# skmhrk1209/VSRD

Measured on AMD Instinct MI355X. Metric: rendered rays/sec (fwd+bwd) per GPU, KITTI-360 376×1408, 16 instances, higher is better.
Workload: dtype f32

## Files before the change

vsrd_amd/csrc/api.hip:

```cpp
#include <cstdio>
#include <cstdlib>
#include "../../include/vsrd_hip.h"
#include "aux_kernels.h"
#include "quad_step.h"
#include "matching.h"
#include "ray_sampling.h"
#include "projection.h"
#include "frame_step.h"
#include "hypernetwork.h"
#include "frame_ingest.h"
#include "frame_labels.h"
#include "frame_group_labels.h"
#include "frame_masks.h"
#include "frame_metrics.h"
#include "frame_log.h"
#include "patch_correlation.h"
#include "launch.h"

namespace {

using namespace vsrd;

constexpr int kMaxBlocks = 16384;

// ... 783 lines not shown
    const bool split = !r.rows && !(config->flags & VSRD_FLAG_STEP_WAVE_PER_RAY) && !wants_samples(config) && (rounds == 2 || rounds == 4) &&
                       (force_split || config->num_rays <= switches().split_max_rays) &&
                       static_cast<size_t>(split_lds_floats(S, N)) * sizeof(float) <= kLdsLimit / 2;
    if (split) {
        const int blocks = config->num_rays < kSplitBlocks ? config->num_rays : kSplitBlocks;
        const int num_waves = blocks * kPairWaves;
        if (static_cast<size_t>(num_waves) * (row + 1) * sizeof(float) > workspace_bytes) return VSRD_E_WORKSPACE;
        if (frames.count > 1 && static_cast<long long>(workspace_bytes) > frames.stride) return VSRD_E_INVALID_ARGUMENT;
        const size_t lds_bytes = static_cast<size_t>(split_lds_floats(S, N)) * sizeof(float);
        const FieldArgs f = field_args(field);
        RenderArgs c = render_args(config);
        c.sh.inv_t = f.inv_t;
        float* partials = static_cast<float*>(workspace);
        float* loss_partials = partials + static_cast<size_t>(num_waves) * row;
        int32_t status = VSRD_OK;
        for_rounds<2, 4>(rounds, [&](auto k) {
            for_bool(frames.count > 1 || header, [&](auto batch) {
                constexpr auto kernel = render_silhouette_split_kernel<decltype(k)::value, decltype(batch)::value>;
                if ((status = opt_in_lds(kernel, lds_bytes)) != VSRD_OK) return;
                hipLaunchKernelGGL(kernel, dim3(blocks, frames.count), dim3(kPairWaves * kWave), lds_bytes, s, f, field->instances, c, origins, directions, u_coarse,
                                   u_fine, targets, instance_weights, loss_scale, labels, partials, loss_partials, header);
            });
        });
        if (status != VSRD_OK) return status;
        if (launch_status() != VSRD_OK) return VSRD_E_LAUNCH;
        hipLaunchKernelGGL(reduce_partials_kernel, dim3(row + 1, frames.count), dim3(256), 0, s, partials, num_waves, row, grad_instances, nullptr, loss_partials, 1, loss,
                           frames.stride, header);
        return launch_status();
    }
    if (frames.count > 1 || header) return VSRD_E_UNSUPPORTED;
    Geometry g;
    if (!plan(r.rows ? static_cast<int>(r.num_groups) : config->num_rays, r.rows ? r.lds_floats : static_cast<size_t>(wave_lds_floats(S, N)) + N + row, &g))
        return VSRD_E_UNSUPPORTED;
#ifdef VSRD_INSTANCE_LDS
    if (r.quad && r.full) g.lds_bytes += static_cast<size_t>(N) * kInstanceStride * sizeof(float);
#endif
    if (!cap_to_workspace(vsrd_workspace_bytes(N, 0), row + 1, r.flag_bytes, &g)) return VSRD_E_WORKSPACE;
    const FieldArgs f = field_args(field);
    RenderArgs c = render_args(config);
    c.sh.inv_t = f.inv_t;
    const int num_waves = g.blocks * (g.threads / kWave);
    float* partials = static_cast<float*>(workspace);
    float* loss_partials = partials + static_cast<size_t>(num_waves) * row;
    unsigned char* redo_flags = reinterpret_cast<unsigned char*>(loss_partials + num_waves);
    int32_t status = VSRD_OK;
    bool known = true;
    if (r.rows) {
        auto launch = [&](auto hot, auto rest) {
            if ((status = opt_in_lds(hot, g.lds_bytes)) != VSRD_OK || (status = opt_in_lds(rest, g.lds_bytes)) != VSRD_OK) return;
            if (hipMemsetAsync(redo_flags, 0, 16, s) != hipSuccess) { status = VSRD_E_LAUNCH; return; }
            launch_hot_then_rest(hot, rest, g, s, f, field->instances, c, origins, directions, u_coarse, u_fine, targets, instance_weights, loss_scale, labels, partials,
                                 loss_partials, redo_flags);
        };
        if (r.quad && r.full) launch(render_silhouette_quad_kernel<4, true, true>, render_silhouette_quad_kernel<4, false, false>);
        else if (r.full) launch(render_silhouette_pair_kernel<4, true, true>, render_silhouette_pair_kernel<4, false, false>);
        else if (r.quad) known = for_rounds<1, 2, 4>(r.rounds, [&](auto k) {
            launch(render_silhouette_quad_kernel<decltype(k)::value, true, false>, render_silhouette_quad_kernel<decltype(k)::value, false, false>); });
        else known = for_rounds<2, 4>(r.rounds, [&](auto k) {
            launch(render_silhouette_pair_kernel<decltype(k)::value, true, false>, render_silhouette_pair_kernel<decltype(k)::value, false, false>); });
    } else {
        known = for_rounds<1, 2, 4>(rounds, [&](auto k) {
            constexpr auto kernel = render_silhouette_kernel<decltype(k)::value>;
            if ((status = opt_in_lds(kernel, g.lds_bytes)) != VSRD_OK) return;
            hipLaunchKernelGGL(kernel, dim3(g.blocks), dim3(g.threads), g.lds_bytes, s, f, field->instances, c, origins, directions, u_coarse, u_fine, targets,
                               instance_weights, loss_scale, labels, partials, loss_partials);
        });
    }
    if (!known) return VSRD_E_UNSUPPORTED;
    if (status != VSRD_OK) return status;
    if (launch_status() != VSRD_OK) return VSRD_E_LAUNCH;
    hipLaunchKernelGGL(reduce_partials_kernel, dim3(row + 1), dim3(256), 0, s, partials, num_waves, row, grad_instances, nullptr, loss_partials, 1, loss);
    return launch_status();
}

static int32_t residual_step_single_kernel(const vsrd_field* field, const vsrd_render_config* config,
                                  const float* origins, const float* directions, const float* u_coarse, const float* u_fine,
                                  const float* targets, const float* instance_weights, float loss_scale, float eikonal_ratio,
                                  void* workspace, size_t workspace_bytes,
                                  float* losses, float* grad_instances, float* grad_mlp_weights, float* labels, void* stream) {
    if (!valid_field(field) || !valid_config(config, true) || !workspace || !losses || !grad_instances || !grad_mlp_weights) return VSRD_E_INVALID_ARGUMENT;
    if (field->mlp_weights == nullptr) return VSRD_E_INVALID_ARGUMENT;
    const int N = field->num_instances;
    if (workspace_bytes < vsrd_workspace_bytes(N, 1)) return VSRD_E_WORKSPACE;
    const hipStream_t s = static_cast<hipStream_t>(stream);
    const int row = N * kGradStride, mlp_row = N * kMlpWeights;
    if (config->num_rays == 0) {
        if (hipMemsetAsync(losses, 0, 2 * sizeof(float), s) != hipSuccess) return VSRD_E_LAUNCH;
        if (hipMemsetAsync(grad_mlp_weights, 0, mlp_row * sizeof(float), s) != hipSuccess) return VSRD_E_LAUNCH;
        return hipMemsetAsync(grad_instances, 0, row * sizeof(float), s) == hipSuccess ? VSRD_OK : VSRD_E_LAUNCH;
    }
    if (!origins || !directions || !targets) return VSRD_E_INVALID_ARGUMENT;
    const int S = config->num_samples;
    const int num_points = 2 * S - 1;
    const int rounds = rounds_for(num_points);
    Geometry g;
    if (!plan(config->num_rays, static_cast<size_t>(residual_step_lds_floats(S, N)), &g)) return VSRD_E_UNSUPPORTED;
    if (g.threads > kResidualWaves * kWave) return VSRD_E_UNSUPPORTED;
    if (g.blocks > kMaxBlocksResidual) g.blocks = kMaxBlocksResidual;
    const FieldArgs f = field_args(field);
    RenderArgs c = render_args(config);
    c.sh.inv_t = f.inv_t;
    const int num_waves = g.blocks * (g.threads / kWave);
    const OneKernelWorkspace w = one_kernel_workspace(workspace, N, true);
    float* loss_partials = w.partials + static_cast<size_t>(num_waves) * row;
    const float eikonal_norm = 1.0f / (static_cast<float>(config->num_rays) * static_cast<float>(num_points));
    const float eikonal_scale = eikonal_ratio * eikonal_norm;
    int32_t status = VSRD_OK;
    const bool known = for_rounds<1, 2, 4>(rounds, [&](auto k) {
// ... 674 lines not shown
```

vsrd_amd/csrc/quad_step.h:

```cpp
#pragma once
#include "render_kernels.h"

namespace vsrd {

constexpr int kQuadRays = 4;
constexpr int kRowLanes = 16;
constexpr int kQuadMaxInstances = 16;
constexpr int kQuadMaxSamples = 64;
constexpr int kPairMaxInstances = 64;
constexpr int kPairMaxSamples = 128;

constexpr int kDppRowShl1 = 0x101, kDppRowShl2 = 0x102, kDppRowShl4 = 0x104, kDppRowShl8 = 0x108;

__device__ __forceinline__ float max_xor16(float v) {
    float a = v, b = v;
    asm volatile("s_nop 1\n\tv_permlane16_swap_b32 %0, %1" : "+v"(a), "+v"(b));
    return fmaxf(a, b);
}
__device__ __forceinline__ float lane_gather(float v, int byte_address) {
    return __builtin_bit_cast(float, __builtin_amdgcn_ds_bpermute(byte_address, __builtin_bit_cast(int, v)));
}

struct RowLanes {
    int lane, row, col;
// ... 169 lines not shown
        }
    }
    if (u_fine == nullptr) {
        const float inv_total = fast_rcp(running + extra_spacing);
#pragma unroll
        for (int k = 0; k < kRoundsS; ++k) {
            const int idx = k * kL + rl.col;
            if (idx < S) {
                const float sorted_u = fminf(spacing[k] * inv_total, 0.99999994f);
                usorted[idx] = sorted_u;
                if (u_fine_out != nullptr && write) u_fine_out[urow + idx] = sorted_u;
            }
        }
    }
    wave_lds_sync();
    if (u_fine != nullptr && !sorted_input) {
#pragma unroll
        for (int k = 0; k < kRoundsS; ++k) {
            if (k * kL >= S) continue;
            const int idx = k * kL + rl.col;
            const bool valid = idx < S;
            const float v = uraw[valid ? idx : 0];
            int rank = 0;
            for (int j = 0; j < S; ++j) {
                const float o = uraw[j];
                rank += ((o < v) || (o == v && j < idx)) ? 1 : 0;
            }
            if (valid) usorted[rank] = v;
        }
        wave_lds_sync();
    }
}

template <bool kStrict>
__device__ __forceinline__ int count_below_64(const float* a, int n, float v) {
    int pos = 0;
#pragma unroll
    for (int stride = 32; stride >= 1; stride >>= 1) {
        const float probe = a[min(pos + stride - 1, n - 1)];
        pos += (kStrict ? (probe < v) : (probe <= v)) ? stride : 0;
    }
    const float probe = a[min(pos, n - 1)];
    pos += (kStrict ? (probe < v) : (probe <= v)) ? 1 : 0;
    return min(pos, n);
}

template <int kL, bool kStrict>
__device__ __forceinline__ int seg_count_below(const float* a, int n, float v) {
    if (kL == kRowLanes) return count_below_64<kStrict>(a, n, v);
    return count_below<kStrict>(a, n, v, search_iterations(n));
}

template <int kL, int kRoundsS>
__device__ __forceinline__ void quad_importance_merge(float* rowbase, int S, const float (&w)[kRoundsS], const RowLanes& rl) {
    float* coarse = rowbase;
    float* fine = rowbase + S;
    float* merged = rowbase + quad_merged_offset(S, kL);
    float* cdf = merged + S;
    float total = 0.0f;
#pragma unroll
    for (int k = 0; k < kRoundsS; ++k) total += seg_sum<kL>(fabsf(w[k]));
    const float denom = fmaxf(total, 1.0e-12f);
    float running = 0.0f;
#pragma unroll
    for (int k = 0; k < kRoundsS; ++k) {
        if (k * kL >= S - 1) continue;
        const int idx = k * kL + rl.col;
        const float inclusive = seg_inclusive_sum<kL>(w[k] / denom) + running;
        if (idx < S - 1) cdf[idx + 1] = inclusive;
        running = lane_gather(inclusive, rl.last);
    }
    if (rl.col == 0) cdf[0] = 0.0f;
    wave_lds_sync();
    float fine_max = -3.0e38f;
#pragma unroll
    for (int k = 0; k < kRoundsS; ++k) {
        if (k * kL >= S) continue;
        const int j = k * kL + rl.col;
        const bool valid = j < S;
        const float u = fine[valid ? j : (S - 1)];
        int upper = seg_count_below<kL, true>(cdf, S, u);
        upper = min(max(upper, 1), S - 1);
        const float c_lo = cdf[upper - 1], c_hi = cdf[upper];
        const float b_lo = coarse[upper - 1], b_hi = coarse[upper];
        const float t = (u - c_lo) / (c_hi - c_lo + 1.0e-6f);
        float sample = torch_lerp(b_lo, b_hi, t);
        const float scan = seg_inclusive_max<kL>(valid ? sample : -3.0e38f);
        sample = fmaxf(scan, fine_max);
        fine_max = fmaxf(fine_max, lane_gather(scan, rl.last));
        wave_lds_sync();
        if (valid) fine[j] = sample;
    }
    wave_lds_sync();
#pragma unroll
    for (int k = 0; k < kRoundsS; ++k) {
        if (k * kL >= S) continue;
        const int j = k * kL + rl.col;
        const bool valid = j < S;
        const int jj = valid ? j : (S - 1);
        const float a = coarse[jj], b = fine[jj];
        const int rank_a = jj + seg_count_below<kL, true>(fine, S, a);
        const int rank_b = jj + seg_count_below<kL, false>(coarse, S, b);
        if (valid) { merged[rank_a] = a; merged[rank_b] = b; }
    }
    wave_lds_sync();
}

struct RowRay { Ray ray; float reach; };
__device__ __forceinline__ RowRay load_row_ray(const float* rp) {
    const float4 a = *reinterpret_cast<const float4*>(rp), b = *reinterpret_cast<const float4*>(rp + 4);
    RowRay r;
    r.ray.ox = a.x; r.ray.oy = a.y; r.ray.oz = a.z; r.ray.rx = a.w; r.ray.ry = b.x; r.ray.rz = b.y; r.reach = b.z;
    return r;
}
__device__ __forceinline__ RayCull row_cull(const float* coef, const RowRay& r) {
    RayCull rc;
    rc.coef = coef;
    rc.c2 = r.ray.rx * r.ray.rx + r.ray.ry * r.ray.ry + r.ray.rz * r.ray.rz;
    rc.rnorm = fast_sqrt(rc.c2);
    rc.reach = r.reach;
    return rc;
}
__device__ __forceinline__ void reload_fence() { asm volatile("" ::: "memory"); }

template <int kL>
__device__ __forceinline__ void quad_ray_setup(const float* __restrict__ instances, int N, int padded, const Ray& r, float* coef, float* rayp, const RowLanes& rl) {
    float amax = 0.0f;
    for (int i = rl.col; i < padded; i += kL) {
        const bool real = i < N;
        const float* p = instances + (real ? i : 0) * kInstanceStride;
        const float ex = r.ox - p[0], ey = r.oy - p[1], ez = r.oz - p[2];
        const float a = ex * ex + ey * ey + ez * ez;
        coef[kCullCoefs * i + 0] = real ? a : 3.0e38f;
        coef[kCullCoefs * i + 1] = real ? 2.0f * (ex * r.rx + ey * r.ry + ez * r.rz) : 0.0f;
        coef[kCullCoefs * i + 2] = real ? fast_sqrt(p[12] * p[12] + p[13] * p[13] + p[14] * p[14]) * (1.0f / (1.0f - kCullSlack)) : 0.0f;
        coef[kCullCoefs * i + 3] = 0.0f;
        amax = fmaxf(amax, real ? a : 0.0f);
    }
    const float reach = fast_sqrt(fmaxf(seg_max<kL>(amax), r.ox * r.ox + r.oy * r.oy + r.oz * r.oz));
    if (rl.col == 0) {
        *reinterpret_cast<float4*>(rayp) = make_float4(r.ox, r.oy, r.oz, r.rx);
        *reinterpret_cast<float4*>(rayp + 4) = make_float4(r.ry, r.rz, reach, 0.0f);
    }
    wave_lds_sync();
}

// ... 286 lines not shown
#endif
            int slot = 0;
            for (unsigned long long todo = st.near[q]; todo != 0ull; todo &= todo - 1ull, ++slot) {
                const int i = __builtin_ctzll(todo);
                if (!((lam_any >> i) & 1ull)) continue;
                acc += coef_own[kCullCoefs * i + 3] * quad_cached_term<(kL > kRowLanes), false, kYaw>(instances, i, slot, cbuf, rl.lane, p.x, p.y, p.z, st.m[q], sh.inv_t);
            }
        } else {
            for (unsigned long long todo = st.near[q] & lam_any; todo != 0ull; todo &= todo - 1ull) {
                const int i = __builtin_ctzll(todo);
                const Instance in = load_instance_block(instances, i);
                acc += coef_own[kCullCoefs * i + 3] * fast_exp(-(box_value<kYaw>(in, p.x, p.y, p.z).d - st.m[q]) * sh.inv_t);
            }
        }
        const float lam_z = p.valid ? acc * st.inv_z[q] : 0.0f;
        UnionValue v;
        v.u = st.m[q] + st.s[q]; v.gx = st.ax[q]; v.gy = st.ay[q]; v.gz = st.az[q];
        const Opacity op = opacity_of(v, rr.ray, p.delta, sh);
        const float alpha = p.valid ? op.alpha : 0.0f;
        const float t = trans_mid[q * kL + rl.col];
        trans_mid[q * kL + rl.col] = p.mid;
        const float wgt = t * alpha;
        const float contrib = lam_z * wgt;
        const float suffix_inclusive = seg_suffix_sum<kL>(contrib, rl);
        const float Q = suffix_inclusive - contrib + suffix_carry;
        suffix_carry += lane_gather(suffix_inclusive, rl.first);
        const float alpha_bar = lam_z * t - Q * fast_rcp(1.0f - alpha);
        const float x_bar = (p.valid && op.xx > 0.0f) ? alpha_bar : 0.0f;
        const float inv_pe = fast_rcp(op.phi_p + sh.eps);
        const float phi_p_bar = x_bar * (op.phi_n + sh.eps) * inv_pe * inv_pe;
        const float phi_n_bar = -x_bar * inv_pe;
        const float sp_bar = phi_p_bar * op.phi_p * (1.0f - op.phi_p) * sh.inv_std;
        const float sn_bar = phi_n_bar * op.phi_n * (1.0f - op.phi_n) * sh.inv_std;
        const float u_bar = sp_bar + sn_bar;
        const float cprime_bar = (sn_bar - sp_bar) * p.delta / 2.0f;
        const float slope = (1.0f - sh.ratio) * ((0.5f - 0.5f * op.cosine > 0.0f) ? 0.5f : 0.0f) + sh.ratio * ((-op.cosine > 0.0f) ? 1.0f : 0.0f);
        const float cos_bar = cprime_bar * slope;
        const float nbx = cos_bar * rr.ray.rx, nby = cos_bar * rr.ray.ry, nbz = cos_bar * rr.ray.rz;
        const float n_dot = op.nx * nbx + op.ny * nby + op.nz * nbz;
        const float gbx = (nbx - op.nx * n_dot) * op.inv_gn, gby = (nby - op.ny * n_dot) * op.inv_gn, gbz = (nbz - op.nz * n_dot) * op.inv_gn;
        const float B = cos_bar * st.c[q];
        const float A = gbx * st.ax[q] + gby * st.ay[q] + gbz * st.az[q];
        st.ax[q] = gbx; st.ay[q] = gby; st.az[q] = gbz;
        st.s[q] = 1.0f + st.s[q] * sh.inv_t;
        c2buf[q * kL + rl.col + 1] = sh.inv_t * (A + wgt * lam_z);
        cbuf[(2 * q) * kWave + rl.lane] = u_bar + sh.inv_t * B;
        cbuf[(2 * q + 1) * kWave + rl.lane] = sh.inv_t * wgt;
        const bool any = (u_bar != 0.0f) || (gbx != 0.0f) || (gby != 0.0f) || (gbz != 0.0f) || (wgt != 0.0f);
        flow |= (__ballot(any) != 0ull) ? (1u << q) : 0u;
    }
    return flow;
}

template <int kL, int kRounds, bool kYaw>
__device__ __forceinline__ void quad_phase_b(const QuadAdjoint<kRounds>& st, const float* __restrict__ instances, const Shading& sh, const float* rayp,
                                             unsigned flow, const float* coef_own, const float* cbuf, const float* mids, const float* c2buf, float (&G)[kL == kRowLanes ? 4 : 16], const RowLanes& rl) {
    const float inv_t = sh.inv_t;
    const Ray ray = load_row_ray(rayp).ray;
    unsigned long long todo = 0ull;
#pragma unroll
    for (int q = 0; q < kRounds; ++q) todo |= ((flow >> q) & 1u) ? st.near[q] : 0ull;
    for (; todo != 0ull; todo &= todo - 1ull) {
        const int i = __builtin_ctzll(todo);
        const Instance in = load_instance_block(instances, i);
        const float lam_i = coef_own[kCullCoefs * i + 3];
        float at0 = 0, at1 = 0, at2 = 0, ad0 = 0, ad1 = 0, ad2 = 0;
        float r00 = 0, r01 = 0, r02 = 0, r10 = 0, r11 = 0, r12 = 0, r20 = 0, r21 = 0, r22 = 0;
#pragma unroll
        for (int q = 0; q < kRounds; ++q) {
            if (!(((st.near[q] >> i) & 1ull) && ((flow >> q) & 1u))) continue;
            const float mid = mids[q * kL + rl.col];
            const float c1 = cbuf[(2 * q) * kWave + rl.lane], c3 = cbuf[(2 * q + 1) * kWave + rl.lane], c2 = c2buf[q * kL + rl.col + 1];
#ifndef VSRD_BOUND_FREE_SELECTORS
            const BoxEval e = eval_box<kYaw>(in, ray.ox + ray.rx * mid, ray.oy + ray.ry * mid, ray.oz + ray.rz * mid);
#else
            BoxEval e = box_value<kYaw>(in, ray.ox + ray.rx * mid, ray.oy + ray.ry * mid, ray.oz + ray.rz * mid);
            e.hx = fmaxf(e.qx, 0.0f) * e.inv; e.hy = fmaxf(e.qy, 0.0f) * e.inv; e.hz = fmaxf(e.qz, 0.0f) * e.inv;
            e.glx = __builtin_copysignf(e.hx, e.px); e.gly = __builtin_copysignf(e.hy, e.py); e.glz = __builtin_copysignf(e.hz, e.pz);
#endif
            const float ds = e.d - st.m[q];
            const float w = fast_exp(-ds * inv_t) * st.inv_z[q];
            const float cc = w * (st.s[q] - ds * inv_t);
            const float gx_ = st.ax[q], gy_ = st.ay[q], gz_ = st.az[q];
            const float rgx = kYaw ? fmaf(in.r20, gz_, in.r00 * gx_) : fmaf(in.r20, gz_, fmaf(in.r10, gy_, in.r00 * gx_));
            const float rgy = kYaw ? gy_ : fmaf(in.r21, gz_, fmaf(in.r11, gy_, in.r01 * gx_));
            const float rgz = kYaw ? fmaf(in.r22, gz_, in.r02 * gx_) : fmaf(in.r22, gz_, fmaf(in.r12, gy_, in.r02 * gx_));
            const float tb = inv_t * (rgx * e.glx + rgy * e.gly + rgz * e.glz);
            const float d_bar = cc * (c1 - tb) + w * (c2 - tb - c3 * lam_i);
            const float gwbx = cc * gx_, gwby = cc * gy_, gwbz = cc * gz_;
            const float glbx = cc * rgx, glby = cc * rgy, glbz = cc * rgz;
#ifndef VSRD_BOUND_FREE_SELECTORS
            const float sx = sign_of(e.px), sy = sign_of(e.py), sz = sign_of(e.pz);
#else
            const float sx = __builtin_copysignf(1.0f, e.px), sy = __builtin_copysignf(1.0f, e.py), sz = __builtin_copysignf(1.0f, e.pz);
#endif
            const float vx = sx * glbx, vy = sy * glby, vz = sz * glbz;
            const float inv_n = box_inverse_norm(e);
            const float hx = fmaxf(e.qx, 0.0f) * inv_n, hy = fmaxf(e.qy, 0.0f) * inv_n, hz = fmaxf(e.qz, 0.0f) * inv_n;
            const float hv = hx * vx + hy * vy + hz * vz;
#ifndef VSRD_BOUND_FREE_SELECTORS
            const float qbx = d_bar * e.hx + ((e.qx > 0.0f) ? (vx - hx * hv) * inv_n : 0.0f);
            const float qby = d_bar * e.hy + ((e.qy > 0.0f) ? (vy - hy * hv) * inv_n : 0.0f);
            const float qbz = d_bar * e.hz + ((e.qz > 0.0f) ? (vz - hz * hv) * inv_n : 0.0f);
#else
            const float qbx = d_bar * e.hx + (vx - hx * hv) * inv_n;
            const float qby = d_bar * e.hy + (vy - hy * hv) * inv_n;
            const float qbz = d_bar * e.hz + (vz - hz * hv) * inv_n;
#endif
            const float pbx = sx * qbx, pby = sy * qby, pbz = sz * qbz;
            ad0 -= qbx; ad1 -= qby; ad2 -= qbz;
            r00 += e.relx * pbx + gwbx * e.glx; r02 += e.relx * pbz + gwbx * e.glz;
            r20 += e.relz * pbx + gwbz * e.glx; r22 += e.relz * pbz + gwbz * e.glz;
            if (!(kYaw && sh.yaw_gradients)) {
                r01 += e.relx * pby + gwbx * e.gly;
                r10 += e.rely * pbx + gwby * e.glx; r11 += e.rely * pby + gwby * e.gly; r12 += e.rely * pbz + gwby * e.glz;
                r21 += e.relz * pby + gwbz * e.gly;
            }
            if (kYaw) {
                at0 -= in.r00 * pbx + in.r02 * pbz; at1 -= pby; at2 -= in.r20 * pbx + in.r22 * pbz;
            } else {
                at0 -= in.r00 * pbx + in.r01 * pby + in.r02 * pbz;
                at1 -= in.r10 * pbx + in.r11 * pby + in.r12 * pbz;
                at2 -= in.r20 * pbx + in.r21 * pby + in.r22 * pbz;
            }
        }
        const float packed[16] = {at0, at1, at2, r00, r01, r02, r10, r11, r12, r20, r21, r22, ad0, ad1, ad2, 0.0f};
        const float mine = wave_reduce16_scatter(packed, rl.lane);
        const float add = ((rl.lane >> 4) == (i & 3)) ? mine : 0.0f;
        if (kL == kRowLanes) {
#pragma unroll
            for (int s = 0; s < 4; ++s) G[s] += ((i >> 2) == s) ? add : 0.0f;
        } else {
            switch (i >> 2) {
#define VSRD_G_CASE(s) case s: G[s] += add; break;
                VSRD_G_CASE(0) VSRD_G_CASE(1) VSRD_G_CASE(2) VSRD_G_CASE(3) VSRD_G_CASE(4) VSRD_G_CASE(5) VSRD_G_CASE(6) VSRD_G_CASE(7)
                VSRD_G_CASE(8) VSRD_G_CASE(9) VSRD_G_CASE(10) VSRD_G_CASE(11) VSRD_G_CASE(12) VSRD_G_CASE(13) VSRD_G_CASE(14) VSRD_G_CASE(15)
#undef VSRD_G_CASE
                default: break;
            }
        }
    }
}

#ifdef VSRD_PHASE_TIMERS
#define VSRD_QUAD_CLOCK_PARAM , PhaseClock& phase_clock
#define VSRD_QUAD_CLOCK_ARG , phase_clock
#else
#define VSRD_QUAD_CLOCK_PARAM
#define VSRD_QUAD_CLOCK_ARG
#endif

template <int kL, int kRoundsS, bool kYaw, bool kRunning>
__device__ __forceinline__ bool quad_step_body(const float* __restrict__ instances, int N, int NP, const RenderArgs& c, const Shading& sh, int first_ray,
                                               const float* __restrict__ origins, const float* __restrict__ directions,
                                               const float* __restrict__ u_coarse, const float* __restrict__ u_fine, bool sorted_input,
                                               const float* __restrict__ targets, const float* __restrict__ instance_weights, float loss_scale,
                                               float* __restrict__ labels_out, float* stage, float* dcache, float* coefs, float* rays,
                                               float (&G)[kL == kRowLanes ? 4 : 16], float& loss_acc, const RowLanes& rl VSRD_QUAD_CLOCK_PARAM) {
    constexpr int kRounds = 2 * kRoundsS;
    constexpr int kSlots = kL == kRowLanes ? 1 : 2;
    VSRD_PHASE(7);
    const int S = c.num_samples;
    const int num_points = 2 * S - 1;
    const int my_ray = first_ray + rl.row;
    const bool alive = my_ray < c.num_rays;
    const int ray = alive ? my_ray : (c.num_rays - 1);
    const long long src = source_row(c, ray);
    float* rowbase = stage + rl.row * quad_row_floats(S, kL);
    float* coef_own = coefs + rl.row * quad_coef_floats(NP);
    const unsigned long long real = NP > N ? ((1ull << N) - 1ull) : ~0ull;
    {
        const long long origin_row = (c.ray_indices && c.rays_per_origin > 0) ? src / c.rays_per_origin : src;
        const float* o = origins + origin_row * c.origin_stride;
        const float* d = directions + src * 3;
        Ray r;
        r.ox = o[0]; r.oy = o[1]; r.oz = o[2]; r.rx = d[0]; r.ry = d[1]; r.rz = d[2];
        quad_ray_setup<kL>(instances, N, NP, r, coef_own, rays + rl.row * kRowRayFloats, rl);
    }
    quad_stage_samples<kL, kRoundsS>(rowbase, c, S, ray, u_coarse, u_fine, sorted_input, rl, c.out_u_coarse, c.out_u_fine, alive);
    VSRD_PHASE(0);
    float w1[kRoundsS];
    if (!quad_pass_one<kL, kRoundsS, kYaw, kRunning>(instances, NP, sh, rays + rl.row * kRowRayFloats, coef_own, rowbase, S, w1, rl, real)) return false;
    VSRD_PHASE(1);
    if (c.out_coarse_weights != nullptr && alive) {
#pragma unroll
        for (int k = 0; k < kRoundsS; ++k)
            if (k * kL + rl.col < S - 1) c.out_coarse_weights[static_cast<size_t>(my_ray) * (S - 1) + k * kL + rl.col] = w1[k];
    }
    float coarse_total = 0.0f;
#pragma unroll
    for (int k = 0; k < kRoundsS; ++k) coarse_total += seg_sum<kL>(w1[k]);
    const bool live = alive && !((c.flags & 2u) && coarse_total == 0.0f);
    const unsigned long long live_lanes = __ballot(live);
    float label[kSlots];
#pragma unroll
    for (int s = 0; s < kSlots; ++s) label[s] = 0.0f;
    unsigned active = 0u;
    int cached_round = -1;
    QuadAdjoint<kRounds> st;
    const int data_row = live ? rl.row : (live_lanes != 0ull ? (__builtin_ctzll(live_lanes) / kL) : rl.row);
    const float* rayp = rays + data_row * kRowRayFloats;
    const float* merged = stage + data_row * quad_row_floats(S, kL) + quad_merged_offset(S, kL);
    float* trans_mid = rowbase;
    if (live_lanes != 0ull) {
        quad_importance_merge<kL, kRoundsS>(rowbase, S, w1, rl);
        if (c.out_distances != nullptr && live) {
            float* dst = c.out_distances + static_cast<size_t>(my_ray) * (2 * S);
            const float* own = rowbase + quad_merged_offset(S, kL);
            for (int idx = rl.col; idx < 2 * S; idx += kL) dst[idx] = own[idx];
        }
        VSRD_PHASE(2);
        if (!quad_forward_sweep<kL, kRounds, kYaw, kRunning>(st, instances, NP, sh, rayp, coefs + data_row * quad_coef_floats(NP), merged, num_points, live, dcache,
                                                         trans_mid, label, active, cached_round, rl, real)) return false;
        VSRD_PHASE(3);
    }
    if (c.out_distances != nullptr && alive && !live && rl.col == 0) c.out_distances[static_cast<size_t>(my_ray) * (2 * S)] = __builtin_nanf("");
    unsigned long long lam_any = 0ull;
    float lam_lane[kSlots];
#pragma unroll
    for (int s = 0; s < kSlots; ++s) {
        const int n = s * kL + rl.col;
        const bool mine = alive && n < N;
        const float lab = live ? label[s] : 0.0f;
        if (labels_out != nullptr && mine) labels_out[static_cast<size_t>(my_ray) * N + n] = lab;
        const float target = mine ? load_target(c, targets, src, n, N) : 0.0f;
        const float weight_lane = mine ? (instance_weights ? instance_weights[n] : 1.0f) : 0.0f;
        const float p = fminf(fmaxf(lab, 1.0e-6f), 1.0f - 1.0e-6f);
        const float bce = -(target * logf(p) + (1.0f - target) * logf(1.0f - p));
        loss_acc += weight_lane * bce;
        const bool inside_clamp = (lab >= 1.0e-6f) && (lab <= 1.0f - 1.0e-6f);
        lam_lane[s] = (live && inside_clamp) ? weight_lane * loss_scale * (p - target) / fmaxf(p * (1.0f - p), 1.0e-12f) : 0.0f;
        unsigned long long any = __ballot(lam_lane[s] != 0.0f);
        any |= any >> 32;
        if (kL == kRowLanes) { any |= any >> 16; any &= 0xFFFFull; } else { any &= 0xFFFFFFFFull; }
        lam_any |= any << (s * kL);
    }
    if (active == 0u || lam_any == 0ull) return true;
#pragma unroll
    for (int s = 0; s < kSlots; ++s)
        if (s * kL + rl.col < N) coef_own[kCullCoefs * (s * kL + rl.col) + 3] = lam_lane[s];
    wave_lds_sync();
    const unsigned flow = quad_reverse_sweep<kL, kRounds, kYaw>(st, instances, sh, rayp, merged, num_points, live, active, lam_any, kRunning ? -1 : cached_round,
                                                            coef_own, dcache, trans_mid, rowbase + quad_merged_offset(S, kL), rl);
    VSRD_PHASE(4);
    if (flow != 0u) quad_phase_b<kL, kRounds, kYaw>(st, instances, sh, rayp, flow, coef_own, dcache, trans_mid, rowbase + quad_merged_offset(S, kL), G, rl);
    VSRD_PHASE(5);
    return true;
}

#ifndef VSRD_QUAD_WAVES_PER_EU
#define VSRD_QUAD_WAVES_PER_EU 4
#endif
template <int kL, int kRoundsS, bool kHot, bool kFull>
__device__ __forceinline__ void silhouette_rows_kernel_body(
    FieldArgs f, const float* __restrict__ instances, RenderArgs c, const float* __restrict__ origins, const float* __restrict__ directions,
    const float* __restrict__ u_coarse, const float* __restrict__ u_fine,
    const float* __restrict__ targets, const float* __restrict__ instance_weights, float loss_scale,
    float* __restrict__ labels_out, float* __restrict__ partials, float* __restrict__ loss_partials, unsigned char* __restrict__ redo_flags) {
    constexpr int kRays = kWave / kL;
    constexpr int kG = kL == kRowLanes ? 4 : 16;
    unsigned* redo_summary = reinterpret_cast<unsigned*>(redo_flags);
    redo_flags += 16;
    if (!kHot && __builtin_amdgcn_readfirstlane(static_cast<int>(redo_summary[1])) != 0 &&
        __builtin_amdgcn_readfirstlane(static_cast<int>(redo_summary[0])) == 0) return;
    apply_device_schedule(f, c);
    extern __shared__ __attribute__((aligned(16))) float lds[];
    const int wave = wave_in_block();
    const int lane0 = lane_id();
    static_assert(kHot || !kFull, "only the hot kernel is instantiated for a full shape");
    if (kFull) c.num_samples = kL * kRoundsS;
    c.ray_indices = nullptr; c.target_columns = nullptr; c.rays_per_origin = 0;
    const int S = c.num_samples;
    const int N = f.num_instances;
    const int NP = kFull ? (kL == kRowLanes ? kQuadMaxInstances : kPairMaxInstances) : N;
    float* stage = lds + wave * quad_lds_floats(S, NP, kL);
    float* dcache = stage + kRays * quad_row_floats(S, kL);
    float* coefs = dcache + quad_cache_floats(S, NP, kL);
    float* rays = coefs + kRays * quad_coef_floats(NP);
    const bool sorted_input = (u_fine != nullptr) && (c.flags & 1u);
    Shading sh = c.sh;
    const FieldBounds bounds = field_bounds(instances, N, f.inv_t, false, c.flags);
    sh.cull = bounds.margin; sh.reach = bounds.reach; sh.yaw = bounds.yaw;
#ifdef VSRD_CULL_INNER
    sh.inner = bounds.inner;
#else
    sh.inner = 0.0f;
#endif
    sh.yaw_gradients = sh.yaw && (c.flags & 1024u) != 0u;
    sh.mlp_bits = 0u;
    sh.mlp_lds = nullptr;
    const bool hot_runs = sh.reach >= 0.0f && sh.yaw;
    if (kHot && !hot_runs) return;
    if (kHot && blockIdx.x == 0 && threadIdx.x == 0) redo_summary[1] = 1u;
#ifdef VSRD_INSTANCE_LDS
    if (kHot && kFull && kL == kRowLanes) {
        float* block = lds + waves_per_block() * quad_lds_floats(S, NP, kL);
        for (int idx = static_cast<int>(threadIdx.x); idx < N * kInstanceStride; idx += static_cast<int>(blockDim.x)) block[idx] = instances[idx];
        __syncthreads();
        instances = block;
    }
#endif
    float loss_acc = 0.0f;
    float G[kG];
#pragma unroll
    for (int s = 0; s < kG; ++s) G[s] = 0.0f;
    const int num_waves = static_cast<int>(gridDim.x) * waves_per_block();
    const int wave_global = static_cast<int>(blockIdx.x) * waves_per_block() + wave;
    const int num_groups = (c.num_rays + kRays - 1) / kRays;
    bool touched = false;
    VSRD_PHASE_CLOCK();
    for (int group = wave_global; group < num_groups; group += num_waves) {
        const int first_ray = group * kRays;
        if (!kHot && hot_runs) {
            if (__builtin_amdgcn_readfirstlane(static_cast<int>(redo_flags[group])) == 0) continue;
            touched = true;
        }
        const RowLanes rl = row_lanes<kL>(opaque_lane_id());
        wave_lds_sync();
        if (kHot) {
            const bool done = quad_step_body<kL, kRoundsS, true, false>(instances, N, NP, c, sh, first_ray, origins, directions, u_coarse, u_fine, sorted_input, targets,
                                                                        instance_weights, loss_scale, labels_out, stage, dcache, coefs, rays, G, loss_acc, rl VSRD_QUAD_CLOCK_ARG);
            if (lane0 == 0) {
                redo_flags[group] = done ? 0 : 1;
                if (!done) atomicAdd(redo_summary, 1u);
            }
        } else {
            bool done = false;
            if (sh.reach >= 0.0f && !hot_runs) {
                done = quad_step_body<kL, kRoundsS, false, false>(instances, N, NP, c, sh, first_ray, origins, directions, u_coarse, u_fine, sorted_input, targets,
                                                                  instance_weights, loss_scale, labels_out, stage, dcache, coefs, rays, G, loss_acc, rl VSRD_QUAD_CLOCK_ARG);
                if (!done) wave_lds_sync();
            }
            if (!done) quad_step_body<kL, kRoundsS, false, true>(instances, N, NP, c, sh, first_ray, origins, directions, u_coarse, u_fine, sorted_input, targets,
                                                                 instance_weights, loss_scale, labels_out, stage, dcache, coefs, rays, G, loss_acc, rl VSRD_QUAD_CLOCK_ARG);
        }
    }
    VSRD_PHASE(7);
    VSRD_PHASE_FLUSH(lane0);
    if (!kHot && hot_runs && !touched) return;
    const bool add = !kHot && hot_runs;
    float* out = partials + static_cast<size_t>(wave_global) * (N * kGradStride);
#pragma unroll
    for (int s = 0; s < kG; ++s)
        if (s * kWave + lane0 < N * kGradStride) out[s * kWave + lane0] = add ? (out[s * kWave + lane0] + G[s]) : G[s];
    const float loss_total = wave_sum(loss_acc);
    if (lane0 == 0) loss_partials[wave_global] = add ? (loss_partials[wave_global] + loss_total * loss_scale) : (loss_total * loss_scale);
}

template <int kRoundsS, bool kHot, bool kFull>
__global__ __launch_bounds__(kBlockThreads, VSRD_QUAD_WAVES_PER_EU) void render_silhouette_quad_kernel(
    FieldArgs f, const float* __restrict__ instances, RenderArgs c, const float* __restrict__ origins, const float* __restrict__ directions,
    const float* __restrict__ u_coarse, const float* __restrict__ u_fine,
    const float* __restrict__ targets, const float* __restrict__ instance_weights, float loss_scale,
    float* __restrict__ labels_out, float* __restrict__ partials, float* __restrict__ loss_partials, unsigned char* __restrict__ redo_flags) {
    silhouette_rows_kernel_body<kRowLanes, kRoundsS, kHot, kFull>(f, instances, c, origins, directions, u_coarse, u_fine, targets, instance_weights, loss_scale, labels_out,
                                                           partials, loss_partials, redo_flags);
}

template <int kL, int kRoundsS, bool kYaw, bool kRunning>
__device__ __forceinline__ bool rows_forward_body(const float* __restrict__ instances, int N, int NP, const RenderArgs& c, const Shading& sh, int first_ray,
                                                  const float* __restrict__ origins, const float* __restrict__ directions,
                                                  const float* __restrict__ u_coarse, const float* __restrict__ u_fine, bool sorted_input,
                                                  float* __restrict__ labels_out, float* __restrict__ distances_out, float* __restrict__ coarse_weights_out,
                                                  float* __restrict__ u_coarse_out, float* __restrict__ u_fine_out,
                                                  float* stage, float* dcache, float* coefs, float* rays, const RowLanes& rl) {
    constexpr int kRounds = 2 * kRoundsS;
    constexpr int kSlots = kL == kRowLanes ? 1 : 2;
    const int S = c.num_samples;
    const int num_points = 2 * S - 1;
    const int my_ray = first_ray + rl.row;
    const bool alive = my_ray < c.num_rays;
    const int ray = alive ? my_ray : (c.num_rays - 1);
    float* rowbase = stage + rl.row * quad_row_floats(S, kL);
    float* coef_own = coefs + rl.row * quad_coef_floats(NP);
    const unsigned long long real = NP > N ? ((1ull << N) - 1ull) : ~0ull;
    {
        const float* o = origins + static_cast<size_t>(ray) * c.origin_stride;
        const float* d = directions + static_cast<size_t>(ray) * 3;
        Ray r;
        r.ox = o[0]; r.oy = o[1]; r.oz = o[2]; r.rx = d[0]; r.ry = d[1]; r.rz = d[2];
        quad_ray_setup<kL>(instances, N, NP, r, coef_own, rays + rl.row * kRowRayFloats, rl);
    }
    quad_stage_samples<kL, kRoundsS>(rowbase, c, S, ray, u_coarse, u_fine, sorted_input, rl, u_coarse_out, u_fine_out, alive);
    float w1[kRoundsS];
    if (!quad_pass_one<kL, kRoundsS, kYaw, kRunning>(instances, NP, sh, rays + rl.row * kRowRayFloats, coef_own, rowbase, S, w1, rl, real)) return false;
    if (coarse_weights_out != nullptr && alive) {
#pragma unroll
        for (int k = 0; k < kRoundsS; ++k)
            if (k * kL + rl.col < S - 1) coarse_weights_out[static_cast<size_t>(my_ray) * (S - 1) + k * kL + rl.col] = w1[k];
    }
    float coarse_total = 0.0f;
#pragma unroll
    for (int k = 0; k < kRoundsS; ++k) coarse_total += seg_sum<kL>(w1[k]);
    const bool live = alive && !((c.flags & 2u) && coarse_total == 0.0f);
    const unsigned long long live_lanes = __ballot(live);
    float label[kSlots];
#pragma unroll
    for (int s = 0; s < kSlots; ++s) label[s] = 0.0f;
    if (live_lanes != 0ull) {
        unsigned active = 0u;
        int cached_round = -1;
        QuadAdjoint<kRounds> st;
        const int data_row = live ? rl.row : (__builtin_ctzll(live_lanes) / kL);
        quad_importance_merge<kL, kRoundsS>(rowbase, S, w1, rl);
        if (!quad_forward_sweep<kL, kRounds, kYaw, kRunning>(st, instances, NP, sh, rays + data_row * kRowRayFloats, coefs + data_row * quad_coef_floats(NP),
                                                              stage + data_row * quad_row_floats(S, kL) + quad_merged_offset(S, kL), num_points, live, dcache,
                                                              rowbase, label, active, cached_round, rl, real)) return false;
    }
#pragma unroll
    for (int s = 0; s < kSlots; ++s) {
        const int n = s * kL + rl.col;
        if (alive && n < N) labels_out[static_cast<size_t>(my_ray) * N + n] = live ? label[s] : 0.0f;
    }
    if (distances_out != nullptr && alive) {
        float* dst = distances_out + static_cast<size_t>(my_ray) * (2 * S);
        if (live) {
            const float* merged = rowbase + quad_merged_offset(S, kL);
            for (int idx = rl.col; idx < 2 * S; idx += kL) dst[idx] = merged[idx];
        } else if (rl.col == 0) {
            dst[0] = __builtin_nanf("");
        }
    }
    return true;
}

template <int kL, int kRoundsS, bool kHot, bool kFull>
__device__ __forceinline__ void hierarchical_rows_kernel_body(
    FieldArgs f, const float* __restrict__ instances, RenderArgs c, const float* __restrict__ origins, const float* __restrict__ directions,
    const float* __restrict__ u_coarse, const float* __restrict__ u_fine, float* __restrict__ labels_out, float* __restrict__ distances_out,
    float* __restrict__ coarse_weights_out, float* __restrict__ u_coarse_out, float* __restrict__ u_fine_out) {
    constexpr int kRays = kWave / kL;
    static_assert(kHot || !kFull, "only the hot kernel is instantiated for a full shape");
    apply_device_schedule(f, c);
    extern __shared__ __attribute__((aligned(16))) float lds[];
    const int wave = wave_in_block();
    if (kFull) c.num_samples = kL * kRoundsS;
    const int S = c.num_samples;
    const int N = f.num_instances;
    const int NP = kFull ? (kL == kRowLanes ? kQuadMaxInstances : kPairMaxInstances) : N;
    float* stage = lds + wave * quad_lds_floats(S, NP, kL);
    float* dcache = stage + kRays * quad_row_floats(S, kL);
    float* coefs = dcache + quad_cache_floats(S, NP, kL);
    float* rays = coefs + kRays * quad_coef_floats(NP);
    const bool sorted_input = (u_fine != nullptr) && (c.flags & 1u);
    Shading sh = c.sh;
    const FieldBounds bounds = field_bounds(instances, N, f.inv_t, false, c.flags);
    sh.cull = bounds.margin; sh.reach = bounds.reach; sh.yaw = bounds.yaw;
#ifdef VSRD_CULL_INNER
    sh.inner = bounds.inner;
#else
    sh.inner = 0.0f;
#endif
    sh.mlp_bits = 0u;
    sh.mlp_lds = nullptr;
    const bool hot_runs = sh.reach >= 0.0f && sh.yaw;
    if (kHot && !hot_runs) return;
    const int num_waves = static_cast<int>(gridDim.x) * waves_per_block();
// ... 157 lines not shown
    const int wave_global = static_cast<int>(blockIdx.x) * waves_per_block() + wave;
    const int num_groups = (c.num_rays + kRays - 1) / kRays;
    bool touched = false;
    for (int group = wave_global; group < num_groups; group += num_waves) {
        const int first_ray = group * kRays;
        if (!kHot && hot_runs) {
            if (__builtin_amdgcn_readfirstlane(static_cast<int>(redo_flags[group])) == 0) continue;
            touched = true;
        }
        const RowLanes rl = row_lanes<kL>(opaque_lane_id());
        wave_lds_sync();
        if (kHot) {
            const bool done = rows_backward_body<kL, kRounds, true, false>(instances, N, NP, c, sh, first_ray, origins, directions, distances, num_distances, grad_labels,
                                                                           stage, dcache, coefs, rays, G, rl);
            if (lane0 == 0) {
                redo_flags[group] = done ? 0 : 1;
                if (!done) atomicAdd(redo_summary, 1u);
            }
        } else {
            bool done = false;
            if (sh.reach >= 0.0f && !hot_runs) {
                done = rows_backward_body<kL, kRounds, false, false>(instances, N, NP, c, sh, first_ray, origins, directions, distances, num_distances, grad_labels,
                                                                     stage, dcache, coefs, rays, G, rl);
                if (!done) wave_lds_sync();
            }
            if (!done) rows_backward_body<kL, kRounds, false, true>(instances, N, NP, c, sh, first_ray, origins, directions, distances, num_distances, grad_labels,
                                                                    stage, dcache, coefs, rays, G, rl);
        }
    }
    if (!kHot && hot_runs && !touched) return;
    const bool add = !kHot && hot_runs;
    float* out = partials + static_cast<size_t>(wave_global) * (N * kGradStride);
#pragma unroll
    for (int s = 0; s < kG; ++s)
        if (s * kWave + lane0 < N * kGradStride) out[s * kWave + lane0] = add ? (out[s * kWave + lane0] + G[s]) : G[s];
}

template <bool kHot, bool kFull>
__global__ __launch_bounds__(kBlockThreads, 4) void render_backward_quad_kernel(
    FieldArgs f, const float* __restrict__ instances, RenderArgs c, const float* __restrict__ origins, const float* __restrict__ directions,
    const float* __restrict__ distances, int num_distances, const float* __restrict__ grad_labels, float* __restrict__ partials, unsigned char* __restrict__ redo_flags) {
    backward_rows_kernel_body<kRowLanes, kHot, kFull>(f, instances, c, origins, directions, distances, num_distances, grad_labels, partials, redo_flags);
}
template <bool kHot, bool kFull>
__global__ __launch_bounds__(kBlockThreads, 3) void render_backward_pair_kernel(
    FieldArgs f, const float* __restrict__ instances, RenderArgs c, const float* __restrict__ origins, const float* __restrict__ directions,
    const float* __restrict__ distances, int num_distances, const float* __restrict__ grad_labels, float* __restrict__ partials, unsigned char* __restrict__ redo_flags) {
    backward_rows_kernel_body<32, kHot, kFull>(f, instances, c, origins, directions, distances, num_distances, grad_labels, partials, redo_flags);
}

#ifndef VSRD_PAIR_WAVES_PER_EU
#define VSRD_PAIR_WAVES_PER_EU 3
#endif
template <int kRoundsS, bool kHot, bool kFull>
__global__ __launch_bounds__(kBlockThreads, VSRD_PAIR_WAVES_PER_EU) void render_silhouette_pair_kernel(
    FieldArgs f, const float* __restrict__ instances, RenderArgs c, const float* __restrict__ origins, const float* __restrict__ directions,
    const float* __restrict__ u_coarse, const float* __restrict__ u_fine,
    const float* __restrict__ targets, const float* __restrict__ instance_weights, float loss_scale,
    float* __restrict__ labels_out, float* __restrict__ partials, float* __restrict__ loss_partials, unsigned char* __restrict__ redo_flags) {
    silhouette_rows_kernel_body<32, kRoundsS, kHot, kFull>(f, instances, c, origins, directions, u_coarse, u_fine, targets, instance_weights, loss_scale, labels_out,
                                                    partials, loss_partials, redo_flags);
}

}
```

Before: 236.8 million.

## Reuse inverse-CDF brackets for merge ranks and specialize yaw-only hot kernels

The importance merge now keeps the CDF bracket index found for each fine sample. When every live lane's sample lies inside its bracket, it computes the merged ranks with a scatter plus a segmented max-scan instead of two binary searches per element, and falls back to the search path otherwise. Separately, the hot full-shape quad and pair kernels get a compile-time yaw-only variant, chosen when the yaw-gradients flag is set, so phase B drops the non-yaw rotation-adjoint accumulations without a runtime check. This adds LDS traffic, register arrays and extra template instantiations, which can add code size and register pressure.

```diff
diff --git a/vsrd_amd/csrc/api.hip b/vsrd_amd/csrc/api.hip
--- a/vsrd_amd/csrc/api.hip
+++ b/vsrd_amd/csrc/api.hip
@@ -859,8 +859,15 @@
             launch_hot_then_rest(hot, rest, g, s, f, field->instances, c, origins, directions, u_coarse, u_fine, targets, instance_weights, loss_scale, labels, partials,
                                  loss_partials, redo_flags);
         };
-        if (r.quad && r.full) launch(render_silhouette_quad_kernel<4, true, true>, render_silhouette_quad_kernel<4, false, false>);
-        else if (r.full) launch(render_silhouette_pair_kernel<4, true, true>, render_silhouette_pair_kernel<4, false, false>);
+#ifndef VSRD_NO_YAW_KERNEL
+        const bool yaw_only = (config->flags & VSRD_FLAG_YAW_GRADIENTS) != 0u;
+#else
+        const bool yaw_only = false;
+#endif
+        if (r.quad && r.full) for_bool(yaw_only, [&](auto y) {
+            launch(render_silhouette_quad_kernel<4, true, true, decltype(y)::value>, render_silhouette_quad_kernel<4, false, false>); });
+        else if (r.full) for_bool(yaw_only, [&](auto y) {
+            launch(render_silhouette_pair_kernel<4, true, true, decltype(y)::value>, render_silhouette_pair_kernel<4, false, false>); });
         else if (r.quad) known = for_rounds<1, 2, 4>(r.rounds, [&](auto k) {
             launch(render_silhouette_quad_kernel<decltype(k)::value, true, false>, render_silhouette_quad_kernel<decltype(k)::value, false, false>); });
         else known = for_rounds<2, 4>(r.rounds, [&](auto k) {
diff --git a/vsrd_amd/csrc/quad_step.h b/vsrd_amd/csrc/quad_step.h
--- a/vsrd_amd/csrc/quad_step.h
+++ b/vsrd_amd/csrc/quad_step.h
@@ -245,7 +245,7 @@
 }
 
 template <int kL, int kRoundsS>
-__device__ __forceinline__ void quad_importance_merge(float* rowbase, int S, const float (&w)[kRoundsS], const RowLanes& rl) {
+__device__ __forceinline__ void quad_importance_merge(float* rowbase, int S, const float (&w)[kRoundsS], const RowLanes& rl, bool votes) {
     float* coarse = rowbase;
     float* fine = rowbase + S;
     float* merged = rowbase + quad_merged_offset(S, kL);
@@ -266,8 +266,15 @@
     if (rl.col == 0) cdf[0] = 0.0f;
     wave_lds_sync();
     float fine_max = -3.0e38f;
+#ifndef VSRD_NO_MERGE_BRACKETS
+    int uppers[kRoundsS];
+    bool bracketed = true;
+#endif
 #pragma unroll
     for (int k = 0; k < kRoundsS; ++k) {
+#ifndef VSRD_NO_MERGE_BRACKETS
+        uppers[k] = 1;
+#endif
         if (k * kL >= S) continue;
         const int j = k * kL + rl.col;
         const bool valid = j < S;
@@ -281,10 +288,55 @@
         const float scan = seg_inclusive_max<kL>(valid ? sample : -3.0e38f);
         sample = fmaxf(scan, fine_max);
         fine_max = fmaxf(fine_max, lane_gather(scan, rl.last));
+#ifndef VSRD_NO_MERGE_BRACKETS
+        uppers[k] = upper;
+        bracketed = bracketed && (!(valid && votes) || (b_lo <= sample && sample < b_hi));
+#endif
         wave_lds_sync();
         if (valid) fine[j] = sample;
     }
     wave_lds_sync();
+#ifndef VSRD_NO_MERGE_BRACKETS
+    if (__ballot(!bracketed) == 0ull) {
+        float* brackets = merged;
+        float* last_of = cdf;
+#pragma unroll
+        for (int k = 0; k < kRoundsS; ++k) {
+            const int j = k * kL + rl.col;
+            if (k * kL < S && j < S) { brackets[j] = static_cast<float>(uppers[k]); last_of[j] = 0.0f; }
+        }
+        wave_lds_sync();
+#pragma unroll
+        for (int k = 0; k < kRoundsS; ++k) {
+            const int j = k * kL + rl.col;
+            if (k * kL < S && j < S) {
+                const float next = brackets[min(j + 1, S - 1)];
+                if (j == S - 1 || next != static_cast<float>(uppers[k])) last_of[uppers[k]] = static_cast<float>(j + 1);
+            }
+        }
+        wave_lds_sync();
+        int rank_a[kRoundsS], rank_b[kRoundsS];
+        float below = 0.0f;
+#pragma unroll
+        for (int k = 0; k < kRoundsS; ++k) {
+            rank_a[k] = rank_b[k] = 0;
+            if (k * kL >= S) continue;
+            const int j = k * kL + rl.col;
+            const float scan = seg_inclusive_max<kL>(j < S ? last_of[j] : 0.0f);
+            rank_a[k] = j + static_cast<int>(fmaxf(scan, below));
+            rank_b[k] = j + uppers[k];
+            below = fmaxf(below, lane_gather(scan, rl.last));
+        }
+        wave_lds_sync();
+#pragma unroll
+        for (int k = 0; k < kRoundsS; ++k) {
+            const int j = k * kL + rl.col;
+            if (k * kL < S && j < S) { merged[rank_a[k]] = coarse[j]; merged[rank_b[k]] = fine[j]; }
+        }
+        wave_lds_sync();
+        return;
+    }
+#endif
 #pragma unroll
     for (int k = 0; k < kRoundsS; ++k) {
         if (k * kL >= S) continue;
@@ -677,7 +729,7 @@
     return flow;
 }
 
-template <int kL, int kRounds, bool kYaw>
+template <int kL, int kRounds, bool kYaw, bool kYawOnly = false>
 __device__ __forceinline__ void quad_phase_b(const QuadAdjoint<kRounds>& st, const float* __restrict__ instances, const Shading& sh, const float* rayp,
                                              unsigned flow, const float* coef_own, const float* cbuf, const float* mids, const float* c2buf, float (&G)[kL == kRowLanes ? 4 : 16], const RowLanes& rl) {
     const float inv_t = sh.inv_t;
@@ -736,7 +788,7 @@
             ad0 -= qbx; ad1 -= qby; ad2 -= qbz;
             r00 += e.relx * pbx + gwbx * e.glx; r02 += e.relx * pbz + gwbx * e.glz;
             r20 += e.relz * pbx + gwbz * e.glx; r22 += e.relz * pbz + gwbz * e.glz;
-            if (!(kYaw && sh.yaw_gradients)) {
+            if (!(kYaw && (kYawOnly || sh.yaw_gradients))) {
                 r01 += e.relx * pby + gwbx * e.gly;
                 r10 += e.rely * pbx + gwby * e.glx; r11 += e.rely * pby + gwby * e.gly; r12 += e.rely * pbz + gwby * e.glz;
                 r21 += e.relz * pby + gwbz * e.gly;
@@ -775,7 +827,7 @@
 #define VSRD_QUAD_CLOCK_ARG
 #endif
 
-template <int kL, int kRoundsS, bool kYaw, bool kRunning>
+template <int kL, int kRoundsS, bool kYaw, bool kRunning, bool kYawOnly = false>
 __device__ __forceinline__ bool quad_step_body(const float* __restrict__ instances, int N, int NP, const RenderArgs& c, const Shading& sh, int first_ray,
                                                const float* __restrict__ origins, const float* __restrict__ directions,
                                                const float* __restrict__ u_coarse, const float* __restrict__ u_fine, bool sorted_input,
@@ -828,7 +880,7 @@
     const float* merged = stage + data_row * quad_row_floats(S, kL) + quad_merged_offset(S, kL);
     float* trans_mid = rowbase;
     if (live_lanes != 0ull) {
-        quad_importance_merge<kL, kRoundsS>(rowbase, S, w1, rl);
+        quad_importance_merge<kL, kRoundsS>(rowbase, S, w1, rl, live);
         if (c.out_distances != nullptr && live) {
             float* dst = c.out_distances + static_cast<size_t>(my_ray) * (2 * S);
             const float* own = rowbase + quad_merged_offset(S, kL);
@@ -868,7 +920,7 @@
     const unsigned flow = quad_reverse_sweep<kL, kRounds, kYaw>(st, instances, sh, rayp, merged, num_points, live, active, lam_any, kRunning ? -1 : cached_round,
                                                             coef_own, dcache, trans_mid, rowbase + quad_merged_offset(S, kL), rl);
     VSRD_PHASE(4);
-    if (flow != 0u) quad_phase_b<kL, kRounds, kYaw>(st, instances, sh, rayp, flow, coef_own, dcache, trans_mid, rowbase + quad_merged_offset(S, kL), G, rl);
+    if (flow != 0u) quad_phase_b<kL, kRounds, kYaw, kYawOnly>(st, instances, sh, rayp, flow, coef_own, dcache, trans_mid, rowbase + quad_merged_offset(S, kL), G, rl);
     VSRD_PHASE(5);
     return true;
 }
@@ -876,7 +928,7 @@
 #ifndef VSRD_QUAD_WAVES_PER_EU
 #define VSRD_QUAD_WAVES_PER_EU 4
 #endif
-template <int kL, int kRoundsS, bool kHot, bool kFull>
+template <int kL, int kRoundsS, bool kHot, bool kFull, bool kYawOnly = false>
 __device__ __forceinline__ void silhouette_rows_kernel_body(
     FieldArgs f, const float* __restrict__ instances, RenderArgs c, const float* __restrict__ origins, const float* __restrict__ directions,
     const float* __restrict__ u_coarse, const float* __restrict__ u_fine,
@@ -893,6 +945,7 @@
     const int wave = wave_in_block();
     const int lane0 = lane_id();
     static_assert(kHot || !kFull, "only the hot kernel is instantiated for a full shape");
+    static_assert(!kYawOnly || (kHot && kFull), "only the hot full-shape kernel is instantiated for VSRD_FLAG_YAW_GRADIENTS");
     if (kFull) c.num_samples = kL * kRoundsS;
     c.ray_indices = nullptr; c.target_columns = nullptr; c.rays_per_origin = 0;
     const int S = c.num_samples;
@@ -943,7 +996,7 @@
         const RowLanes rl = row_lanes<kL>(opaque_lane_id());
         wave_lds_sync();
         if (kHot) {
-            const bool done = quad_step_body<kL, kRoundsS, true, false>(instances, N, NP, c, sh, first_ray, origins, directions, u_coarse, u_fine, sorted_input, targets,
+            const bool done = quad_step_body<kL, kRoundsS, true, false, kYawOnly>(instances, N, NP, c, sh, first_ray, origins, directions, u_coarse, u_fine, sorted_input, targets,
                                                                         instance_weights, loss_scale, labels_out, stage, dcache, coefs, rays, G, loss_acc, rl VSRD_QUAD_CLOCK_ARG);
             if (lane0 == 0) {
                 redo_flags[group] = done ? 0 : 1;
@@ -972,13 +1025,13 @@
     if (lane0 == 0) loss_partials[wave_global] = add ? (loss_partials[wave_global] + loss_total * loss_scale) : (loss_total * loss_scale);
 }
 
-template <int kRoundsS, bool kHot, bool kFull>
+template <int kRoundsS, bool kHot, bool kFull, bool kYawOnly = false>
 __global__ __launch_bounds__(kBlockThreads, VSRD_QUAD_WAVES_PER_EU) void render_silhouette_quad_kernel(
     FieldArgs f, const float* __restrict__ instances, RenderArgs c, const float* __restrict__ origins, const float* __restrict__ directions,
     const float* __restrict__ u_coarse, const float* __restrict__ u_fine,
     const float* __restrict__ targets, const float* __restrict__ instance_weights, float loss_scale,
     float* __restrict__ labels_out, float* __restrict__ partials, float* __restrict__ loss_partials, unsigned char* __restrict__ redo_flags) {
-    silhouette_rows_kernel_body<kRowLanes, kRoundsS, kHot, kFull>(f, instances, c, origins, directions, u_coarse, u_fine, targets, instance_weights, loss_scale, labels_out,
+    silhouette_rows_kernel_body<kRowLanes, kRoundsS, kHot, kFull, kYawOnly>(f, instances, c, origins, directions, u_coarse, u_fine, targets, instance_weights, loss_scale, labels_out,
                                                            partials, loss_partials, redo_flags);
 }
 
@@ -1027,7 +1080,7 @@
         int cached_round = -1;
         QuadAdjoint<kRounds> st;
         const int data_row = live ? rl.row : (__builtin_ctzll(live_lanes) / kL);
-        quad_importance_merge<kL, kRoundsS>(rowbase, S, w1, rl);
+        quad_importance_merge<kL, kRoundsS>(rowbase, S, w1, rl, live);
         if (!quad_forward_sweep<kL, kRounds, kYaw, kRunning>(st, instances, NP, sh, rays + data_row * kRowRayFloats, coefs + data_row * quad_coef_floats(NP),
                                                               stage + data_row * quad_row_floats(S, kL) + quad_merged_offset(S, kL), num_points, live, dcache,
                                                               rowbase, label, active, cached_round, rl, real)) return false;
@@ -1291,13 +1344,13 @@
 #ifndef VSRD_PAIR_WAVES_PER_EU
 #define VSRD_PAIR_WAVES_PER_EU 3
 #endif
-template <int kRoundsS, bool kHot, bool kFull>
+template <int kRoundsS, bool kHot, bool kFull, bool kYawOnly = false>
 __global__ __launch_bounds__(kBlockThreads, VSRD_PAIR_WAVES_PER_EU) void render_silhouette_pair_kernel(
     FieldArgs f, const float* __restrict__ instances, RenderArgs c, const float* __restrict__ origins, const float* __restrict__ directions,
     const float* __restrict__ u_coarse, const float* __restrict__ u_fine,
     const float* __restrict__ targets, const float* __restrict__ instance_weights, float loss_scale,
     float* __restrict__ labels_out, float* __restrict__ partials, float* __restrict__ loss_partials, unsigned char* __restrict__ redo_flags) {
-    silhouette_rows_kernel_body<32, kRoundsS, kHot, kFull>(f, instances, c, origins, directions, u_coarse, u_fine, targets, instance_weights, loss_scale, labels_out,
+    silhouette_rows_kernel_body<32, kRoundsS, kHot, kFull, kYawOnly>(f, instances, c, origins, directions, u_coarse, u_fine, targets, instance_weights, loss_scale, labels_out,
                                                     partials, loss_partials, redo_flags);
 }
 
```

Result: faster. 241.5 million (median of 6 runs) (+2.0%).
